# snap-research/MMVID

Hardware: AMD Instinct MI355X
Metric: video-tokens/sec training step, 8-frame 128px text-to-video (higher is better)
Workload: dtype bf16

## Files before the change

mmvid_amd/csrc/attn.hip:

```cpp
#include <type_traits>

#include "../../include/mmvid_hip.h"
#include "gemm_core.h"
#include "prof.h"

namespace {
using mmvid_core::blds16;
using mmvid_core::dma_publish_barrier;
using mmvid_core::make_rsrc;
using mmvid_core::rsrc_t;
using mmvid_core::bf16x4_t;
using mmvid_core::ds_read_tr16;
using mmvid_core::lds_addr;
using mmvid_core::lgkm_wait_tied;
using mmvid_core::xcd_remap;

struct MaskSpec {
    int mode;
    int r0, c0, r1, c1;
};

__device__ __forceinline__ bool is_masked(const MaskSpec& m, int q, int key, int L) {
    const bool pad = key >= L;
    const bool causal = (m.mode == 1) & (key > q);
    const bool rows = (m.mode == 2) & (((q == m.r0) & (key < m.c0)) | ((q == m.r1) & (key < m.c1)));
    return pad | causal | rows;
}

constexpr int TILE = 64 * 128;
constexpr int ROWS_PER_BLOCK = 128;
constexpr float RESCALE_THR = 8.0f;

__device__ __forceinline__ int swz(int row) {
    const int x = (row >> 1) & 7;
    return ((x & 1) << 2) | (x >> 1);
}

struct FastDiv {
    uint32_t d, m;
};
static FastDiv make_fastdiv(int d) {
    FastDiv f;
    f.d = (uint32_t)d, f.m = d > 1 ? (uint32_t)((1ull << 32) / (uint32_t)d) + 1u : 0u;
    return f;
}
__device__ __forceinline__ uint32_t fdiv(uint32_t n, FastDiv f) { return f.d == 1 ? n : __umulhi(n, f.m); }

struct TileStage {
    rsrc_t rsrc;
    uint32_t voff[2], rowbytes;
    __device__ __forceinline__ void init(const bf16_t* slice, long ld, int L, int wave, int lane) {
        rsrc = make_rsrc(slice, (uint32_t)(((long)(L - 1) * ld + 64) * 2));
        rowbytes = (uint32_t)ld * 2u;
#pragma unroll
        for (int jj = 0; jj < 2; ++jj) {
            const int row = (wave * 2 + jj) * 8 + (lane >> 3);
            const int chunk = (lane & 7) ^ swz(row);
            voff[jj] = (uint32_t)row * rowbytes + (uint32_t)chunk * 16u;
        }
    }
    __device__ __forceinline__ void issue(int p0, char* tile, int wave) const {
#pragma unroll
        for (int jj = 0; jj < 2; ++jj) blds16(rsrc, voff[jj], (uint32_t)p0 * rowbytes, tile + (wave * 2 + jj) * 1024);
    }
};

struct RowLane {
    uint32_t o[4];
};
__device__ __forceinline__ RowLane row_lane_offs(int lane) {
    const int l32 = lane & 31, h = lane >> 5;
    RowLane r;
#pragma unroll
    for (int s = 0; s < 4; ++s) r.o[s] = (uint32_t)(l32 * 128 + (((2 * s + h) ^ swz(l32)) << 4));
    return r;
}
template <int SS, int S>
__device__ __forceinline__ bf16x8_t row_frag(const char* tile, const RowLane& rl) {
    return *reinterpret_cast<const bf16x8_t*>(tile + SS * 4096 + rl.o[S]);
}
struct TrLane {
    uint32_t o[2][2];
};
__device__ __forceinline__ TrLane tr_lane_offs(int lane) {
    const int G = lane >> 4, si = lane & 15;
    const int rowl = 4 * (G >> 1) + (si >> 2);
    const int cl = 2 * (G & 1) + ((si & 3) >> 1);
    const int x0 = (rowl >> 1) & 1, x1 = (rowl >> 2) & 1;
    TrLane t;
#pragma unroll
    for (int dt = 0; dt < 2; ++dt)
#pragma unroll
        for (int x2 = 0; x2 < 2; ++x2) t.o[dt][x2] = (uint32_t)(rowl * 128 + ((4 * (dt ^ x0) + (cl ^ x1 ^ (2 * x2))) << 4) + 8 * (si & 1));
    return t;
}
__device__ __forceinline__ TrLane tr_lane_at(const TrLane& t, uint32_t base) {
    TrLane a;
#pragma unroll
    for (int dt = 0; dt < 2; ++dt)
#pragma unroll
        for (int x2 = 0; x2 < 2; ++x2) a.o[dt][x2] = t.o[dt][x2] + base;
    return a;
}
template <int DT, int SS, int M, int OFF>
__device__ __forceinline__ bf16x8_t tr_frag(const TrLane& tl) {
    const bf16x4_t lo = ds_read_tr16<OFF + (32 * SS + 16 * M) * 128>(tl.o[DT][0]);
    const bf16x4_t hi = ds_read_tr16<OFF + (32 * SS + 16 * M + 8) * 128>(tl.o[DT][1]);
    return __builtin_shufflevector(lo, hi, 0, 1, 2, 3, 4, 5, 6, 7);
}
template <int SS, int OFF>
__device__ __forceinline__ void tr_frags4(const TrLane& tl, bf16x8_t (&f)[4]) {
    f[0] = tr_frag<0, SS, 0, OFF>(tl), f[1] = tr_frag<1, SS, 0, OFF>(tl);
    f[2] = tr_frag<0, SS, 1, OFF>(tl), f[3] = tr_frag<1, SS, 1, OFF>(tl);
}
__device__ __forceinline__ bf16x8_t pack_half(const f32x16& a, int m) {
    const int o = 8 * m;
    const uint4 u = make_uint4(pack_bf2(a[o], a[o + 1]), pack_bf2(a[o + 2], a[o + 3]), pack_bf2(a[o + 4], a[o + 5]),
                               pack_bf2(a[o + 6], a[o + 7]));
    return __builtin_bit_cast(bf16x8_t, u);
}
__device__ __forceinline__ f32x16 mfma32(bf16x8_t a, bf16x8_t b, f32x16 c) {
    return __builtin_amdgcn_mfma_f32_32x32x16_bf16(a, b, c, 0, 0, 0);
}
__device__ __forceinline__ f32x16 mfma32z(bf16x8_t a, bf16x8_t b) {
    const f32x16 z = {0.f, 0.f, 0.f, 0.f, 0.f, 0.f, 0.f, 0.f, 0.f, 0.f, 0.f, 0.f, 0.f, 0.f, 0.f, 0.f};
    return __builtin_amdgcn_mfma_f32_32x32x16_bf16(a, b, z, 0, 0, 0);
}
__device__ __forceinline__ f32x16 zero16() {
    f32x16 z;
#pragma unroll
    for (int r = 0; r < 16; ++r) z[r] = 0.f;
    return z;
}
__device__ __forceinline__ constexpr int acc_row(int r, int h) { return (r & 3) + 8 * (r >> 2) + 4 * h; }
__device__ __forceinline__ float fast_exp2(float x) { return __builtin_amdgcn_exp2f(x); }
__device__ __forceinline__ float max16(const f32x16& a) {
    float m0, m1;
    asm("v_max3_f32 %0, %1, %2, %3" : "=v"(m0) : "v"(a[0]), "v"(a[1]), "v"(a[2]));
    asm("v_max3_f32 %0, %1, %2, %3" : "=v"(m1) : "v"(a[3]), "v"(a[4]), "v"(a[5]));
    asm("v_max3_f32 %0, %1, %2, %3" : "=v"(m0) : "v"(m0), "v"(a[6]), "v"(a[7]));
    asm("v_max3_f32 %0, %1, %2, %3" : "=v"(m1) : "v"(m1), "v"(a[8]), "v"(a[9]));
    asm("v_max3_f32 %0, %1, %2, %3" : "=v"(m0) : "v"(m0), "v"(a[10]), "v"(a[11]));
    asm("v_max3_f32 %0, %1, %2, %3" : "=v"(m1) : "v"(m1), "v"(a[12]), "v"(a[13]));
    asm("v_max3_f32 %0, %1, %2, %3" : "=v"(m0) : "v"(m0), "v"(a[14]), "v"(a[15]));
    asm("v_max_f32 %0, %1, %2" : "=v"(m0) : "v"(m0), "v"(m1));
    return m0;
}
__device__ __forceinline__ float half_max(float v) {
    const uint32_t u = __float_as_uint(v);
    const auto r = __builtin_amdgcn_permlane32_swap(u, u, false, false);
    float m;
    asm("v_max_f32 %0, %1, %2" : "=v"(m) : "v"(__uint_as_float(r[0])), "v"(__uint_as_float(r[1])));
    return m;
}
__device__ __forceinline__ float half_sum(float v) {
    const uint32_t u = __float_as_uint(v);
    const auto r = __builtin_amdgcn_permlane32_swap(u, u, false, false);
    return __uint_as_float(r[0]) + __uint_as_float(r[1]);
}
__device__ __forceinline__ float exp2_affine_sum(f32x16& a, float sc, float nb) {
    float s0 = 0.f, s1 = 0.f;
#pragma unroll
    for (int i = 0; i < 8; ++i) {
        float x, y;
        asm("v_fma_f32 %0, %1, %2, %3" : "=v"(x) : "v"(a[2 * i]), "v"(sc), "v"(nb));
        asm("v_fma_f32 %0, %1, %2, %3" : "=v"(y) : "v"(a[2 * i + 1]), "v"(sc), "v"(nb));
        x = fast_exp2(x), y = fast_exp2(y);
        a[2 * i] = x, a[2 * i + 1] = y;
        asm("v_add_f32 %0, %1, %2" : "=v"(s0) : "v"(s0), "v"(x));
        asm("v_add_f32 %0, %1, %2" : "=v"(s1) : "v"(s1), "v"(y));
    }
    return s0 + s1;
}
__device__ __forceinline__ void mask_pad_keys(f32x16& s, int kl) {
#pragma unroll
    for (int r = 0; r < 16; ++r) s[r] = (acc_row(r, 0) >= kl) ? -INFINITY : s[r];
}

__device__ __forceinline__ uint4 widen_pair(uint2 lo, uint2 hi) {
    const auto a = __builtin_amdgcn_permlane32_swap(lo.x, hi.x, false, false);
    const auto b = __builtin_amdgcn_permlane32_swap(lo.y, hi.y, false, false);
    return make_uint4(a[0], b[0], a[1], b[1]);
}
__device__ __forceinline__ void store_row64(bf16_t* row_ptr, const f32x16 (&acc)[2], float scale, int h) {
#pragma unroll
    for (int dt = 0; dt < 2; ++dt)
#pragma unroll
        for (int k = 0; k < 2; ++k) {
            uint2 pc[2];
#pragma unroll
            for (int u = 0; u < 2; ++u) {
                const int g4 = 2 * k + u;
                pc[u] = make_uint2(pack_bf2(acc[dt][4 * g4] * scale, acc[dt][4 * g4 + 1] * scale),
                                   pack_bf2(acc[dt][4 * g4 + 2] * scale, acc[dt][4 * g4 + 3] * scale));
            }
            *reinterpret_cast<uint4*>(row_ptr + 32 * dt + 16 * k + 8 * h) = widen_pair(pc[0], pc[1]);
        }
}

__device__ __forceinline__ void colsum_rows64(const f32x16 (&acc)[2], float scale, bool live, float* dst, int lane) {
    float cs[32];
#pragma unroll
    for (int dt = 0; dt < 2; ++dt)
#pragma unroll
        for (int r = 0; r < 16; ++r) cs[16 * dt + r] = live ? acc[dt][r] * scale : 0.f;
#pragma unroll
    for (int s = 0; s < 5; ++s) {
        const int m = 1 << s;
        const bool up = (lane & m) != 0;
#pragma unroll
        for (int t = 0; t < (16 >> s); ++t) {
            const float keep = up ? cs[2 * t + 1] : cs[2 * t];
            const float send = up ? cs[2 * t] : cs[2 * t + 1];
            cs[t] = keep + __shfl_xor(send, m, 64);
        }
    }
    const int c = lane & 31, h = lane >> 5;
    unsafeAtomicAdd(dst + 32 * (c >> 4) + 8 * ((c >> 2) & 3) + 4 * h + (c & 3), cs[0]);
}

struct BlockCoords {
    int rt, hd, b;
};
__device__ __forceinline__ BlockCoords block_coords(FastDiv nrt, FastDiv H) {
    BlockCoords c;
    const uint32_t id = (uint32_t)xcd_remap(blockIdx.x, gridDim.x);
    const uint32_t bh = fdiv(id, nrt);
    c.rt = (int)(id - bh * nrt.d);
    c.b = (int)fdiv(bh, H);
    c.hd = (int)(bh - (uint32_t)c.b * H.d);
    return c;
}

template <int V>
using ic = std::integral_constant<int, V>;

template <bool KEYLEN>
__global__ __launch_bounds__(256, 3) void attn_fwd_kernel(const bf16_t* __restrict__ qkv, long ld, int L, int H, int E, FastDiv nrt_d,
                                                           FastDiv h_d, float scale_log2, MaskSpec mask, bf16_t* __restrict__ out,
                                                           long ldo, float* __restrict__ lse2, const int32_t* __restrict__ key_len) {
    __shared__ __attribute__((aligned(16))) char smem[2][2 * TILE];
    const int tid = threadIdx.x, lane = tid & 63, wave = __builtin_amdgcn_readfirstlane(tid >> 6), l32 = lane & 31, h = lane >> 5;
    const BlockCoords bc = block_coords(nrt_d, h_d);
    const int qt = bc.rt, hd = bc.hd, b = bc.b;
    const int Lk = KEYLEN ? min(max(key_len[b], 1), L) : L;
    const bf16_t* Kbase = qkv + (long)b * L * ld + E + hd * 64;
    const bf16_t* Vbase = Kbase + E;
    const RowLane rl = row_lane_offs(lane);
    const TrLane trv = tr_lane_at(tr_lane_offs(lane), lds_addr(smem[0] + TILE));
    const int q_wave0 = qt * ROWS_PER_BLOCK + wave * 32;
    const int q = q_wave0 + l32;
    const int qc = q < L ? q : L - 1;
    const bool wave_active = q_wave0 < L;
    bf16x8_t qf[4];
    {
        const bf16_t* Qp = qkv + ((long)b * L + qc) * ld + hd * 64;
#pragma unroll
        for (int s = 0; s < 4; ++s) qf[s] = *reinterpret_cast<const bf16x8_t*>(Qp + 16 * s + 8 * h);
    }
    int kv_end = Lk;
    if (mask.mode == 1) {
        const int blk_end = (qt + 1) * ROWS_PER_BLOCK;
        if (blk_end < L) kv_end = blk_end;
    }
    const int t_begin = 0, t_end = (kv_end + 63) >> 6;

    TileStage stK, stV;
    stK.init(Kbase, ld, Lk, wave, lane), stV.init(Vbase, ld, Lk, wave, lane);
    stK.issue(t_begin * 64, smem[0], wave), stV.issue(t_begin * 64, smem[0] + TILE, wave);

    float m_run = -INFINITY, nref = 0.f, thr_raw = -INFINITY, lsum = 0.f;
    const float inv_scale_log2 = 1.0f / scale_log2;
    f32x16 oacc[2] = {zero16(), zero16()};
    const int row_kmax = mask.mode != 2 ? 0
                                        : max((mask.r0 >= q_wave0 && mask.r0 < q_wave0 + 32) ? mask.c0 : 0,
                                              (mask.r1 >= q_wave0 && mask.r1 < q_wave0 + 32) ? mask.c1 : 0);
    int lo = (row_kmax + 63) >> 6, hi = min(t_end - 1, Lk >> 6);
    if (mask.mode == 1) hi = min(hi, (q_wave0 + 1) >> 6);
    lo = max(lo, t_begin);
    lo += (lo - t_begin) & 1;
    if (lo >= t_end) lo = t_end;
    hi = hi > lo ? lo + ((hi - lo) & ~1) : lo;
    const int kl0 = Lk - 4 * h;

    auto tile = [&](auto st_c, auto plain_c, int t) {
        constexpr int ST = decltype(st_c)::value;
        constexpr bool PLAIN = decltype(plain_c)::value != 0;
        constexpr int VOFF = ST * 2 * TILE;
        const char* Kt = smem[ST];
        char* nxt = smem[ST ^ 1];
        const bool more = PLAIN || t + 1 < t_end;
        const bool two = PLAIN || t * 64 + 32 < Lk;
        f32x16 sv[2];
        auto s_mfmas = [&](auto ss_c) {
            constexpr int SS = decltype(ss_c)::value;
            sv[SS] = mfma32z(row_frag<SS, 0>(Kt, rl), qf[0]);
            sv[SS] = mfma32(row_frag<SS, 1>(Kt, rl), qf[1], sv[SS]);
            sv[SS] = mfma32(row_frag<SS, 2>(Kt, rl), qf[2], sv[SS]);
            sv[SS] = mfma32(row_frag<SS, 3>(Kt, rl), qf[3], sv[SS]);
        };
        s_mfmas(ic<0>{});
        if constexpr (PLAIN) s_mfmas(ic<1>{});
        if (more) {
            __builtin_amdgcn_sched_barrier(0);
            stK.issue((t + 1) * 64, nxt, wave), stV.issue((t + 1) * 64, nxt + TILE, wave);
        }
        auto sub = [&](auto ss_c) {
            constexpr int SS = decltype(ss_c)::value;
            const int key0 = t * 64 + 32 * SS;
            f32x16& s = sv[SS];
            if constexpr (!PLAIN) mfma_settle(s);
            bf16x8_t vt[4];
            tr_frags4<SS, VOFF>(trv, vt);
            if constexpr (!PLAIN) {
                if ((mask.mode == 1 && key0 + 31 > q_wave0) || key0 < row_kmax) {
#pragma unroll
                    for (int r = 0; r < 16; ++r) s[r] = is_masked(mask, q, key0 + acc_row(r, h), Lk) ? -INFINITY : s[r];
                } else if (key0 + 32 > Lk) {
                    mask_pad_keys(s, kl0 - key0);
                }
            }
            const float mx_raw = half_max(max16(s));
            if (__any(mx_raw > thr_raw)) {
                const float m_new = fmaxf(m_run, mx_raw * scale_log2);
                const float m_ref = (m_new == -INFINITY) ? 0.f : m_new;
                const float alpha = fast_exp2(m_run - m_ref);
                lsum *= alpha;
#pragma unroll
                for (int dt = 0; dt < 2; ++dt)
#pragma unroll
                    for (int r = 0; r < 16; ++r) oacc[dt][r] *= alpha;
                m_run = m_new, nref = -m_ref, thr_raw = (m_new + RESCALE_THR) * inv_scale_log2;
            }
            lsum += exp2_affine_sum(s, scale_log2, nref);
            bf16x8_t pf[2] = {pack_half(s, 0), pack_half(s, 1)};
            lgkm_wait_tied<0>(vt[0], vt[1], vt[2], vt[3], pf[0], pf[1]);
            oacc[0] = mfma32(vt[0], pf[0], oacc[0]);
            oacc[1] = mfma32(vt[1], pf[0], oacc[1]);
            oacc[0] = mfma32(vt[2], pf[1], oacc[0]);
            oacc[1] = mfma32(vt[3], pf[1], oacc[1]);
        };
        sub(ic<0>{});
        if (two) {
            if constexpr (!PLAIN) s_mfmas(ic<1>{});
            sub(ic<1>{});
        }
    };
    if (!wave_active) {
        for (int t = t_begin; t < t_end; ++t) {
            dma_publish_barrier();
            char* nxt = smem[(t + 1 - t_begin) & 1];
            if (t + 1 < t_end) stK.issue((t + 1) * 64, nxt, wave), stV.issue((t + 1) * 64, nxt + TILE, wave);
        }
        return;
    }
#pragma unroll 1
    for (int ph = 0; ph < 2; ++ph) {
        const int a = ph == 0 ? t_begin : hi, z = ph == 0 ? lo : t_end;
#pragma unroll 1
        for (int t = a; t < z; ++t) {
            dma_publish_barrier();
            if ((t - t_begin) & 1)
                tile(ic<1>{}, ic<0>{}, t);
            else
                tile(ic<0>{}, ic<0>{}, t);
        }
        if (ph == 0) {
#pragma unroll 1
            for (int t = lo; t < hi; t += 2) {
                dma_publish_barrier();
                tile(ic<0>{}, ic<1>{}, t);
                dma_publish_barrier();
                tile(ic<1>{}, ic<1>{}, t + 1);
            }
        }
    }
    lsum = half_sum(lsum);
    mfma_settle(oacc[0]), mfma_settle(oacc[1]);
    if (q < L) {
        store_row64(out + ((long)b * L + q) * ldo + hd * 64, oacc, 1.0f / lsum, h);
        if (h == 0 && (!KEYLEN || lse2)) lse2[((long)b * H + hd) * L + q] = m_run + log2f(lsum);
    }
}

__global__ __launch_bounds__(256, 3) void attn_bwd_dq_kernel(const bf16_t* __restrict__ qkv, long ld, const bf16_t* __restrict__ O, long ldo,
                                                              const bf16_t* __restrict__ dO, long lddo, const float* __restrict__ lse2,
                                                              float* __restrict__ delta, int L, int H, int E, FastDiv nrt_d, FastDiv h_d,
                                                              float scale, float scale_log2, MaskSpec mask, bf16_t* __restrict__ dqkv,
                                                              long ldg, float* __restrict__ dbias) {
    __shared__ __attribute__((aligned(16))) char smem[2][2 * TILE];
    const int tid = threadIdx.x, lane = tid & 63, wave = __builtin_amdgcn_readfirstlane(tid >> 6), l32 = lane & 31, h = lane >> 5;
    const BlockCoords bc = block_coords(nrt_d, h_d);
    const int qt = bc.rt, hd = bc.hd, b = bc.b;
    const bf16_t* Kbase = qkv + (long)b * L * ld + E + hd * 64;
    const bf16_t* Vbase = Kbase + E;
    const RowLane rl = row_lane_offs(lane);
    const TrLane trk = tr_lane_at(tr_lane_offs(lane), lds_addr(smem[0]));
    const int q_wave0 = qt * ROWS_PER_BLOCK + wave * 32;
    const int q = q_wave0 + l32;
    const int qc = q < L ? q : L - 1;
    const bool wave_active = q_wave0 < L;
    bf16x8_t qf[4], dof[4];
    float neg_lse, my_delta;
    {
        const bf16_t* Qp = qkv + ((long)b * L + qc) * ld + hd * 64;
        const bf16_t* dOp = dO + ((long)b * L + qc) * lddo + hd * 64;
        const bf16_t* Op = O + ((long)b * L + qc) * ldo + hd * 64;
        uint4 o4[4];
#pragma unroll
        for (int s = 0; s < 4; ++s) {
            qf[s] = *reinterpret_cast<const bf16x8_t*>(Qp + 16 * s + 8 * h);
            dof[s] = *reinterpret_cast<const bf16x8_t*>(dOp + 16 * s + 8 * h);
            o4[s] = *reinterpret_cast<const uint4*>(Op + 16 * s + 8 * h);
        }
        neg_lse = -lse2[((long)b * H + hd) * L + qc];
        float d = 0.f;
#pragma unroll
        for (int s = 0; s < 4; ++s) {
            const uint4 d4 = __builtin_bit_cast(uint4, dof[s]);
            d += (bf_lo(o4[s].x) * bf_lo(d4.x) + bf_hi(o4[s].x) * bf_hi(d4.x)) + (bf_lo(o4[s].y) * bf_lo(d4.y) + bf_hi(o4[s].y) * bf_hi(d4.y)) +
                 (bf_lo(o4[s].z) * bf_lo(d4.z) + bf_hi(o4[s].z) * bf_hi(d4.z)) + (bf_lo(o4[s].w) * bf_lo(d4.w) + bf_hi(o4[s].w) * bf_hi(d4.w));
        }
        my_delta = half_sum(d);
        if (h == 0 && q < L) delta[((long)b * H + hd) * L + q] = my_delta;
    }
    int kv_end = L;
    if (mask.mode == 1) {
        const int blk_end = (qt + 1) * ROWS_PER_BLOCK;
        if (blk_end < L) kv_end = blk_end;
    }
    const int t_begin = 0, t_end = (kv_end + 63) >> 6;

    TileStage sk, sv;
    sk.init(Kbase, ld, L, wave, lane), sv.init(Vbase, ld, L, wave, lane);
    sk.issue(t_begin * 64, smem[0], wave), sv.issue(t_begin * 64, smem[0] + TILE, wave);

    f32x16 dq[2] = {zero16(), zero16()};
    const int row_kmax = mask.mode != 2 ? 0
                                        : max((mask.r0 >= q_wave0 && mask.r0 < q_wave0 + 32) ? mask.c0 : 0,
                                              (mask.r1 >= q_wave0 && mask.r1 < q_wave0 + 32) ? mask.c1 : 0);
    int lo = (row_kmax + 63) >> 6, hi = min(t_end - 1, L >> 6);
    if (mask.mode == 1) hi = min(hi, (q_wave0 + 1) >> 6);
    lo = max(lo, t_begin);
    lo += (lo - t_begin) & 1;
    if (lo >= t_end) lo = t_end;
    hi = hi > lo ? lo + ((hi - lo) & ~1) : lo;

    auto tile = [&](auto st_c, auto plain_c, int t) {
        constexpr int ST = decltype(st_c)::value;
        constexpr bool PLAIN = decltype(plain_c)::value != 0;
        constexpr int KOFF = ST * 2 * TILE;
        const char* Kt = smem[ST];
        const char* Vt = Kt + TILE;
        char* nxt = smem[ST ^ 1];
        const bool more = PLAIN || t + 1 < t_end;
        auto sub = [&](auto ss_c) {
            constexpr int SS = decltype(ss_c)::value;
            const int key0 = t * 64 + 32 * SS;
            f32x16 s = mfma32z(row_frag<SS, 0>(Kt, rl), qf[0]);
            f32x16 dp = mfma32z(row_frag<SS, 0>(Vt, rl), dof[0]);
            s = mfma32(row_frag<SS, 1>(Kt, rl), qf[1], s), dp = mfma32(row_frag<SS, 1>(Vt, rl), dof[1], dp);
            s = mfma32(row_frag<SS, 2>(Kt, rl), qf[2], s), dp = mfma32(row_frag<SS, 2>(Vt, rl), dof[2], dp);
            s = mfma32(row_frag<SS, 3>(Kt, rl), qf[3], s), dp = mfma32(row_frag<SS, 3>(Vt, rl), dof[3], dp);
            if (SS == 0 && more) {
                __builtin_amdgcn_sched_barrier(0);
                sk.issue((t + 1) * 64, nxt, wave), sv.issue((t + 1) * 64, nxt + TILE, wave);
            }
            mfma_settle(s), mfma_settle(dp);
            bf16x8_t kt4[4];
            tr_frags4<SS, KOFF>(trk, kt4);
            if constexpr (!PLAIN) {
                if ((mask.mode == 1 && key0 + 31 > q_wave0) || key0 < row_kmax) {
#pragma unroll
                    for (int r = 0; r < 16; ++r) s[r] = is_masked(mask, q, key0 + acc_row(r, h), L) ? -INFINITY : s[r];
                }
                if (key0 + 32 > L) {
#pragma unroll
                    for (int r = 0; r < 16; ++r) s[r] = (key0 + acc_row(r, h) >= L) ? -INFINITY : s[r];
                }
            }
            (void)exp2_affine_sum(s, scale_log2, neg_lse);
#pragma unroll
            for (int r = 0; r < 16; ++r) s[r] *= dp[r] - my_delta;
            bf16x8_t dsf[2] = {pack_half(s, 0), pack_half(s, 1)};
            lgkm_wait_tied<0>(kt4[0], kt4[1], kt4[2], kt4[3], dsf[0], dsf[1]);
            dq[0] = mfma32(kt4[0], dsf[0], dq[0]);
            dq[1] = mfma32(kt4[1], dsf[0], dq[1]);
            dq[0] = mfma32(kt4[2], dsf[1], dq[0]);
            dq[1] = mfma32(kt4[3], dsf[1], dq[1]);
        };
        sub(ic<0>{});
        if (PLAIN || t * 64 + 32 < L) sub(ic<1>{});
    };
    if (!wave_active) {
        for (int t = t_begin; t < t_end; ++t) {
            dma_publish_barrier();
            char* nxt = smem[(t + 1 - t_begin) & 1];
            if (t + 1 < t_end) sk.issue((t + 1) * 64, nxt, wave), sv.issue((t + 1) * 64, nxt + TILE, wave);
        }
        return;
    }
#pragma unroll 1
    for (int ph = 0; ph < 2; ++ph) {
        const int a = ph == 0 ? t_begin : hi, z = ph == 0 ? lo : t_end;
#pragma unroll 1
        for (int t = a; t < z; ++t) {
            dma_publish_barrier();
            if ((t - t_begin) & 1)
                tile(ic<1>{}, ic<0>{}, t);
            else
                tile(ic<0>{}, ic<0>{}, t);
        }
        if (ph == 0) {
#pragma unroll 1
            for (int t = lo; t < hi; t += 2) {
                dma_publish_barrier();
                tile(ic<0>{}, ic<1>{}, t);
                dma_publish_barrier();
                tile(ic<1>{}, ic<1>{}, t + 1);
            }
        }
    }
    mfma_settle(dq[0]), mfma_settle(dq[1]);
    if (q < L) store_row64(dqkv + ((long)b * L + q) * ldg + hd * 64, dq, scale, h);
    if (dbias) colsum_rows64(dq, scale, q < L, dbias + hd * 64, lane);
}

constexpr int DKV_BUF = 2 * TILE + 512;

__global__ __launch_bounds__(256, 2) void attn_bwd_dkv_kernel(const bf16_t* __restrict__ qkv, long ld, const bf16_t* __restrict__ dO, long lddo,
                                                               const float* __restrict__ lse2, const float* __restrict__ delta, int L, int H,
                                                               int E, FastDiv nrt_d, FastDiv h_d, float scale, float scale_log2, MaskSpec mask,
                                                               bf16_t* __restrict__ dqkv, long ldg, float* __restrict__ dbias) {
    __shared__ __attribute__((aligned(16))) char dsm[2][DKV_BUF];
    const int tid = threadIdx.x, lane = tid & 63, wave = __builtin_amdgcn_readfirstlane(tid >> 6), l32 = lane & 31, h = lane >> 5;
    const BlockCoords bc = block_coords(nrt_d, h_d);
    const int kt = bc.rt, hd = bc.hd, b = bc.b;
    const bf16_t* Qbase = qkv + (long)b * L * ld + hd * 64;
    const bf16_t* dObase = dO + (long)b * L * lddo + hd * 64;
    const float* lse_b = lse2 + ((long)b * H + hd) * L;
    const float* del_b = delta + ((long)b * H + hd) * L;
    const int nq_tiles = (L + 63) >> 6;
    const RowLane rl = row_lane_offs(lane);
    const TrLane tr0 = tr_lane_offs(lane);
    const TrLane trq = tr_lane_at(tr0, lds_addr(dsm[0])), trdo = tr_lane_at(tr0, lds_addr(dsm[0] + TILE));
    const int key_wave0 = kt * ROWS_PER_BLOCK + wave * 32;
    const int key = key_wave0 + l32;
    const bool wave_active = key_wave0 < L;
    bf16x8_t kf[4], vf[4];
    {
        const int keyc = key < L ? key : L - 1;
        const bf16_t* Kp = qkv + ((long)b * L + keyc) * ld + E + hd * 64;
        const bf16_t* Vp = Kp + E;
#pragma unroll
        for (int s = 0; s < 4; ++s) {
            kf[s] = *reinterpret_cast<const bf16x8_t*>(Kp + 16 * s + 8 * h);
            vf[s] = *reinterpret_cast<const bf16x8_t*>(Vp + 16 * s + 8 * h);
        }
    }
    auto load_stat = [&](int t) -> float {
        if (tid >= 128) return 0.f;
        const int qq = t * 64 + (tid & 63);
        if (tid < 64) return qq < L ? -lse_b[qq] : -INFINITY;
        return qq < L ? del_b[qq] : 0.f;
    };
    const int t_begin = (mask.mode == 1) ? (kt * ROWS_PER_BLOCK) >> 6 : 0, t_end = nq_tiles;

    TileStage sq, sdo;
    sq.init(Qbase, ld, L, wave, lane), sdo.init(dObase, lddo, L, wave, lane);
    sq.issue(t_begin * 64, dsm[0], wave), sdo.issue(t_begin * 64, dsm[0] + TILE, wave);
    float stat = load_stat(t_begin);
    if (tid < 128) reinterpret_cast<float*>(dsm[0] + 2 * TILE)[tid] = stat;

    f32x16 dk[2] = {zero16(), zero16()}, dv[2] = {zero16(), zero16()};
    const bool rows_hit0 = mask.mode == 2 && key_wave0 < mask.c0, rows_hit1 = mask.mode == 2 && key_wave0 < mask.c1;

    auto tile = [&](auto st_c, int t) {
        constexpr int ST = decltype(st_c)::value;
        constexpr int OFF = ST * DKV_BUF;
        const char* Qt = dsm[ST];
        const char* dOt = Qt + TILE;
        const float* st_nlse = reinterpret_cast<const float*>(Qt + 2 * TILE);
        const float* st_del = st_nlse + 64;
        char* nx = dsm[ST ^ 1];
        const bool more = t + 1 < t_end;
        dma_publish_barrier();
        if (!wave_active) {
            if (more) {
                sq.issue((t + 1) * 64, nx, wave), sdo.issue((t + 1) * 64, nx + TILE, wave);
                stat = load_stat(t + 1);
                if (tid < 128) reinterpret_cast<float*>(nx + 2 * TILE)[tid] = stat;
            }
            return;
        }
        auto sub = [&](auto ss_c) {
            constexpr int SS = decltype(ss_c)::value;
            const int q0 = t * 64 + 32 * SS;
            f32x16 s = mfma32z(row_frag<SS, 0>(Qt, rl), kf[0]);
            f32x16 dp = mfma32z(row_frag<SS, 0>(dOt, rl), vf[0]);
            s = mfma32(row_frag<SS, 1>(Qt, rl), kf[1], s), dp = mfma32(row_frag<SS, 1>(dOt, rl), vf[1], dp);
            s = mfma32(row_frag<SS, 2>(Qt, rl), kf[2], s), dp = mfma32(row_frag<SS, 2>(dOt, rl), vf[2], dp);
            s = mfma32(row_frag<SS, 3>(Qt, rl), kf[3], s), dp = mfma32(row_frag<SS, 3>(dOt, rl), vf[3], dp);
            if (SS == 0 && more) {
                __builtin_amdgcn_sched_barrier(0);
                sq.issue((t + 1) * 64, nx, wave), sdo.issue((t + 1) * 64, nx + TILE, wave);
                stat = load_stat(t + 1);
            }
            mfma_settle(s), mfma_settle(dp);
            bf16x8_t dot4[4], qt4[4];
            tr_frags4<SS, OFF>(trdo, dot4);
            tr_frags4<SS, OFF>(trq, qt4);
            bool nm = mask.mode == 1 && key_wave0 + 31 > q0;
            nm = nm || (rows_hit0 && mask.r0 >= q0 && mask.r0 < q0 + 32) || (rows_hit1 && mask.r1 >= q0 && mask.r1 < q0 + 32);
            if (nm) {
#pragma unroll
                for (int r = 0; r < 16; ++r) s[r] = is_masked(mask, q0 + acc_row(r, h), key, L) ? -INFINITY : s[r];
            }
            const f32x2 sc2 = {scale_log2, scale_log2};
#pragma unroll
            for (int g4 = 0; g4 < 4; ++g4) {
                const int ql = 32 * SS + 8 * g4 + 4 * h;
                const float4 l4 = *reinterpret_cast<const float4*>(st_nlse + ql);
                const float4 d4 = *reinterpret_cast<const float4*>(st_del + ql);
                f32x2 a = {s[4 * g4], s[4 * g4 + 1]}, c = {s[4 * g4 + 2], s[4 * g4 + 3]};
                a = __builtin_elementwise_fma(a, sc2, (f32x2){l4.x, l4.y});
                c = __builtin_elementwise_fma(c, sc2, (f32x2){l4.z, l4.w});
                const float p0 = fast_exp2(a[0]), p1 = fast_exp2(a[1]), p2 = fast_exp2(c[0]), p3 = fast_exp2(c[1]);
                s[4 * g4] = p0, s[4 * g4 + 1] = p1, s[4 * g4 + 2] = p2, s[4 * g4 + 3] = p3;
                dp[4 * g4] = p0 * (dp[4 * g4] - d4.x);
                dp[4 * g4 + 1] = p1 * (dp[4 * g4 + 1] - d4.y);
                dp[4 * g4 + 2] = p2 * (dp[4 * g4 + 2] - d4.z);
                dp[4 * g4 + 3] = p3 * (dp[4 * g4 + 3] - d4.w);
            }
            bf16x8_t pf[2] = {pack_half(s, 0), pack_half(s, 1)};
            bf16x8_t dsf[2] = {pack_half(dp, 0), pack_half(dp, 1)};
            lgkm_wait_tied<8>(dot4[0], dot4[1], dot4[2], dot4[3], pf[0], pf[1]);
            dv[0] = mfma32(dot4[0], pf[0], dv[0]);
            dv[1] = mfma32(dot4[1], pf[0], dv[1]);
            dv[0] = mfma32(dot4[2], pf[1], dv[0]);
            dv[1] = mfma32(dot4[3], pf[1], dv[1]);
            lgkm_wait_tied<0>(qt4[0], qt4[1], qt4[2], qt4[3], dsf[0], dsf[1]);
            dk[0] = mfma32(qt4[0], dsf[0], dk[0]);
            dk[1] = mfma32(qt4[1], dsf[0], dk[1]);
            dk[0] = mfma32(qt4[2], dsf[1], dk[0]);
            dk[1] = mfma32(qt4[3], dsf[1], dk[1]);
        };
        sub(ic<0>{});
        if (t * 64 + 32 < L) sub(ic<1>{});
        if (more && tid < 128) reinterpret_cast<float*>(nx + 2 * TILE)[tid] = stat;
    };
    for (int t = t_begin; t < t_end; t += 2) {
        tile(ic<0>{}, t);
        if (t + 1 >= t_end) break;
        tile(ic<1>{}, t + 1);
    }
    if (!wave_active) return;
    mfma_settle(dk[0]), mfma_settle(dk[1]), mfma_settle(dv[0]), mfma_settle(dv[1]);
    if (key < L) {
        bf16_t* kp = dqkv + ((long)b * L + key) * ldg + E + hd * 64;
        store_row64(kp, dk, scale, h);
        store_row64(kp + E, dv, 1.0f, h);
    }
    if (dbias) {
        colsum_rows64(dk, scale, key < L, dbias + E + hd * 64, lane);
        colsum_rows64(dv, 1.0f, key < L, dbias + 2 * E + hd * 64, lane);
    }
}

static MaskSpec make_mask(int mode, int r0, int c0, int r1, int c1) {
    MaskSpec m;
    m.mode = mode, m.r0 = r0, m.c0 = c0, m.r1 = r1, m.c1 = c1;
    return m;
}

}

#define ATTN_COMMON_CHECKS(name)                                                                            \
    MMVID_REQUIRE(B > 0 && L > 0 && H > 0 && E == H * 64, name ": need E == H*64 (head_dim 64), got E=%d H=%d", E, H); \
    MMVID_REQUIRE(mask_mode >= 0 && mask_mode <= 2, name ": mask_mode %d", mask_mode);                             \
    MMVID_REQUIRE((int64_t)cdiv(L, ROWS_PER_BLOCK) * H * B * (H > 64 ? H : 64) < (1ll << 31), name ": too many (batch, head, row block) units")

extern "C" int mmvid_attention_fwd(const void* qkv, int64_t ld, int B, int L, int H, int E, float scale, int mask_mode,
                                   int r0, int c0, int r1, int c1, void* out, int64_t ldo, float* lse2, void* stream) {
    MMVID_REQUIRE(qkv && out && lse2, "attention_fwd: null pointer");
    ATTN_COMMON_CHECKS("attention_fwd");
    MMVID_REQUIRE(ld % 8 == 0 && ldo % 8 == 0 && ((uintptr_t)out & 15) == 0, "attention_fwd: leading dims must be multiples of 8, out 16-byte aligned");
    MMVID_REQUIRE((int64_t)L * ld * 2 < (1ll << 31), "attention_fwd: one batch entry of qkv must be smaller than 2 GiB");
    hipStream_t s = (hipStream_t)stream;
    MmvidProfScope prof(PROF_ATTN_FWD, 4.0 * B * H * (double)L * L * 64, s);
    const int nrt = cdiv(L, ROWS_PER_BLOCK), nblocks = nrt * H * B;
    const FastDiv nrt_d = make_fastdiv(nrt), h_d = make_fastdiv(H);
    const MaskSpec m = make_mask(mask_mode, r0, c0, r1, c1);
    hipLaunchKernelGGL(attn_fwd_kernel<false>, dim3(nblocks), dim3(256), 0, s, (const bf16_t*)qkv, (long)ld, L, H, E, nrt_d, h_d,
                       scale * 1.4426950408889634f, m, (bf16_t*)out, (long)ldo, lse2, (const int32_t*)nullptr);
    MMVID_LAUNCH_CHECK("attention_fwd");
    return MMVID_OK;
}

extern "C" int mmvid_attention_fwd_keylen(const void* qkv, int64_t ld, int B, int L, int H, int E, float scale, const int32_t* key_len,
                                          void* out, int64_t ldo, float* lse2, void* stream) {
    MMVID_REQUIRE(qkv && out && key_len, "attention_fwd_keylen: null pointer");
    const int mask_mode = 0;
    ATTN_COMMON_CHECKS("attention_fwd_keylen");
    MMVID_REQUIRE(ld % 8 == 0 && ldo % 8 == 0 && ((uintptr_t)out & 15) == 0,
                  "attention_fwd_keylen: leading dims must be multiples of 8, out 16-byte aligned");
    MMVID_REQUIRE((int64_t)L * ld * 2 < (1ll << 31), "attention_fwd_keylen: one batch entry of qkv must be smaller than 2 GiB");
    hipStream_t s = (hipStream_t)stream;
    MmvidProfScope prof(PROF_ATTN_FWD, 4.0 * B * H * (double)L * L * 64, s);
    const int nrt = cdiv(L, ROWS_PER_BLOCK), nblocks = nrt * H * B;
    const FastDiv nrt_d = make_fastdiv(nrt), h_d = make_fastdiv(H);
    hipLaunchKernelGGL(attn_fwd_kernel<true>, dim3(nblocks), dim3(256), 0, s, (const bf16_t*)qkv, (long)ld, L, H, E, nrt_d, h_d,
                       scale * 1.4426950408889634f, make_mask(0, -1, 0, -1, 0), (bf16_t*)out, (long)ldo, lse2, key_len);
    MMVID_LAUNCH_CHECK("attention_fwd_keylen");
    return MMVID_OK;
}

extern "C" int mmvid_attention_bwd(const void* qkv, int64_t ld, const void* O, int64_t ldo, const void* dO, int64_t lddo,
                                   const float* lse2, float* delta, int B, int L, int H, int E, float scale,
                                   int mask_mode, int r0, int c0, int r1, int c1, void* dqkv, int64_t ldg,
                                   void* stream) {
    return mmvid_attention_bwd_bias(qkv, ld, O, ldo, dO, lddo, lse2, delta, B, L, H, E, scale, mask_mode, r0, c0, r1, c1, dqkv, ldg,
                                    nullptr, stream);
}

extern "C" int mmvid_attention_bwd_bias(const void* qkv, int64_t ld, const void* O, int64_t ldo, const void* dO, int64_t lddo,
                                        const float* lse2, float* delta, int B, int L, int H, int E, float scale,
                                        int mask_mode, int r0, int c0, int r1, int c1, void* dqkv, int64_t ldg,
                                        float* dbias, void* stream) {
    MMVID_REQUIRE(qkv && O && dO && lse2 && delta && dqkv, "attention_bwd: null pointer");
    ATTN_COMMON_CHECKS("attention_bwd");
    MMVID_REQUIRE(ld % 8 == 0 && ldo % 8 == 0 && lddo % 8 == 0 && ldg % 8 == 0 && ((uintptr_t)dqkv & 15) == 0,
                  "attention_bwd: leading dims must be multiples of 8, dqkv 16-byte aligned");
    MMVID_REQUIRE((int64_t)L * ld * 2 < (1ll << 31) && (int64_t)L * lddo * 2 < (1ll << 31),
                  "attention_bwd: one batch entry of qkv / dO must be smaller than 2 GiB");
    hipStream_t s = (hipStream_t)stream;
    const MaskSpec m = make_mask(mask_mode, r0, c0, r1, c1);
    const float sl2 = scale * 1.4426950408889634f;
    MmvidProfScope prof(PROF_ATTN_BWD, 10.0 * B * H * (double)L * L * 64, s);
    const int nrt = cdiv(L, ROWS_PER_BLOCK), nblocks = nrt * H * B;
    const FastDiv nrt_d = make_fastdiv(nrt), h_d = make_fastdiv(H);
    hipLaunchKernelGGL(attn_bwd_dq_kernel, dim3(nblocks), dim3(256), 0, s, (const bf16_t*)qkv, (long)ld, (const bf16_t*)O, (long)ldo,
                       (const bf16_t*)dO, (long)lddo, lse2, delta, L, H, E, nrt_d, h_d, scale, sl2, m, (bf16_t*)dqkv, (long)ldg, dbias);
    hipLaunchKernelGGL(attn_bwd_dkv_kernel, dim3(nblocks), dim3(256), 0, s, (const bf16_t*)qkv, (long)ld, (const bf16_t*)dO, (long)lddo, lse2,
                       delta, L, H, E, nrt_d, h_d, scale, sl2, m, (bf16_t*)dqkv, (long)ldg, dbias);
    MMVID_LAUNCH_CHECK("attention_bwd");
    return MMVID_OK;
}
```

Baseline: 215,900.

## Fold softmax stats into MFMA accumulator init and raise dkv occupancy

The dK/dV backward kernel now seeds the S and dP MFMA accumulators with the per-row -lse/scale and -delta values. The exponent then becomes a single multiply and exp, and dS becomes a single multiply, which removes the per-element FMA/subtract work and the separate stat loads in the inner loop. Launch bounds go from 2 to 3 blocks per SIMD, the Q-transpose read is deferred to cut register pressure, and the tile-stage DMA uses one offset register for two 32-row halves. The risks are inline asm scheduling (s_nop hazard handling), register spills at the higher occupancy target, and a small precision change from dividing lse by scale.

```diff
diff --git a/mmvid_amd/csrc/attn.hip b/mmvid_amd/csrc/attn.hip
--- a/mmvid_amd/csrc/attn.hip
+++ b/mmvid_amd/csrc/attn.hip
@@ -48,20 +48,17 @@
 
 struct TileStage {
     rsrc_t rsrc;
-    uint32_t voff[2], rowbytes;
+    uint32_t voff, rowbytes;
     __device__ __forceinline__ void init(const bf16_t* slice, long ld, int L, int wave, int lane) {
         rsrc = make_rsrc(slice, (uint32_t)(((long)(L - 1) * ld + 64) * 2));
         rowbytes = (uint32_t)ld * 2u;
-#pragma unroll
-        for (int jj = 0; jj < 2; ++jj) {
-            const int row = (wave * 2 + jj) * 8 + (lane >> 3);
-            const int chunk = (lane & 7) ^ swz(row);
-            voff[jj] = (uint32_t)row * rowbytes + (uint32_t)chunk * 16u;
-        }
+        const int row = wave * 8 + (lane >> 3);
+        const int chunk = (lane & 7) ^ swz(row);
+        voff = (uint32_t)row * rowbytes + (uint32_t)chunk * 16u;
     }
     __device__ __forceinline__ void issue(int p0, char* tile, int wave) const {
-#pragma unroll
-        for (int jj = 0; jj < 2; ++jj) blds16(rsrc, voff[jj], (uint32_t)p0 * rowbytes, tile + (wave * 2 + jj) * 1024);
+        blds16(rsrc, voff, (uint32_t)p0 * rowbytes, tile + wave * 1024);
+        blds16(rsrc, voff, (uint32_t)(p0 + 32) * rowbytes, tile + (wave + 4) * 1024);
     }
 };
 
@@ -528,10 +525,22 @@
 
 constexpr int DKV_BUF = 2 * TILE + 512;
 
-__global__ __launch_bounds__(256, 2) void attn_bwd_dkv_kernel(const bf16_t* __restrict__ qkv, long ld, const bf16_t* __restrict__ dO, long lddo,
+template <int SS>
+__device__ __forceinline__ f32x16 row_consts(const float* st, int h) {
+    f32x16 a;
+#pragma unroll
+    for (int g4 = 0; g4 < 4; ++g4) {
+        const float4 v = *reinterpret_cast<const float4*>(st + 32 * SS + 8 * g4 + 4 * h);
+        a[4 * g4] = v.x, a[4 * g4 + 1] = v.y, a[4 * g4 + 2] = v.z, a[4 * g4 + 3] = v.w;
+    }
+    return a;
+}
+
+__global__ __launch_bounds__(256, 3) void attn_bwd_dkv_kernel(const bf16_t* __restrict__ qkv, long ld, const bf16_t* __restrict__ dO, long lddo,
                                                                const float* __restrict__ lse2, const float* __restrict__ delta, int L, int H,
-                                                               int E, FastDiv nrt_d, FastDiv h_d, float scale, float scale_log2, MaskSpec mask,
-                                                               bf16_t* __restrict__ dqkv, long ldg, float* __restrict__ dbias) {
+                                                               int E, FastDiv nrt_d, FastDiv h_d, float scale, float scale_log2,
+                                                               float inv_scale_log2, MaskSpec mask, bf16_t* __restrict__ dqkv, long ldg,
+                                                               float* __restrict__ dbias) {
     __shared__ __attribute__((aligned(16))) char dsm[2][DKV_BUF];
     const int tid = threadIdx.x, lane = tid & 63, wave = __builtin_amdgcn_readfirstlane(tid >> 6), l32 = lane & 31, h = lane >> 5;
     const BlockCoords bc = block_coords(nrt_d, h_d);
@@ -542,8 +551,7 @@
     const float* del_b = delta + ((long)b * H + hd) * L;
     const int nq_tiles = (L + 63) >> 6;
     const RowLane rl = row_lane_offs(lane);
-    const TrLane tr0 = tr_lane_offs(lane);
-    const TrLane trq = tr_lane_at(tr0, lds_addr(dsm[0])), trdo = tr_lane_at(tr0, lds_addr(dsm[0] + TILE));
+    const TrLane trq = tr_lane_at(tr_lane_offs(lane), lds_addr(dsm[0]));
     const int key_wave0 = kt * ROWS_PER_BLOCK + wave * 32;
     const int key = key_wave0 + l32;
     const bool wave_active = key_wave0 < L;
@@ -561,8 +569,8 @@
     auto load_stat = [&](int t) -> float {
         if (tid >= 128) return 0.f;
         const int qq = t * 64 + (tid & 63);
-        if (tid < 64) return qq < L ? -lse_b[qq] : -INFINITY;
-        return qq < L ? del_b[qq] : 0.f;
+        if (tid < 64) return qq < L ? -lse_b[qq] * inv_scale_log2 : -INFINITY;
+        return qq < L ? -del_b[qq] : 0.f;
     };
     const int t_begin = (mask.mode == 1) ? (kt * ROWS_PER_BLOCK) >> 6 : 0, t_end = nq_tiles;
 
@@ -581,7 +589,7 @@
         const char* Qt = dsm[ST];
         const char* dOt = Qt + TILE;
         const float* st_nlse = reinterpret_cast<const float*>(Qt + 2 * TILE);
-        const float* st_del = st_nlse + 64;
+        const float* st_ndel = st_nlse + 64;
         char* nx = dsm[ST ^ 1];
         const bool more = t + 1 < t_end;
         dma_publish_barrier();
@@ -596,8 +604,8 @@
         auto sub = [&](auto ss_c) {
             constexpr int SS = decltype(ss_c)::value;
             const int q0 = t * 64 + 32 * SS;
-            f32x16 s = mfma32z(row_frag<SS, 0>(Qt, rl), kf[0]);
-            f32x16 dp = mfma32z(row_frag<SS, 0>(dOt, rl), vf[0]);
+            f32x16 s = row_consts<SS>(st_nlse, h), dp = row_consts<SS>(st_ndel, h);
+            s = mfma32(row_frag<SS, 0>(Qt, rl), kf[0], s), dp = mfma32(row_frag<SS, 0>(dOt, rl), vf[0], dp);
             s = mfma32(row_frag<SS, 1>(Qt, rl), kf[1], s), dp = mfma32(row_frag<SS, 1>(dOt, rl), vf[1], dp);
             s = mfma32(row_frag<SS, 2>(Qt, rl), kf[2], s), dp = mfma32(row_frag<SS, 2>(dOt, rl), vf[2], dp);
             s = mfma32(row_frag<SS, 3>(Qt, rl), kf[3], s), dp = mfma32(row_frag<SS, 3>(dOt, rl), vf[3], dp);
@@ -607,33 +615,26 @@
                 stat = load_stat(t + 1);
             }
             mfma_settle(s), mfma_settle(dp);
-            bf16x8_t dot4[4], qt4[4];
-            tr_frags4<SS, OFF>(trdo, dot4);
-            tr_frags4<SS, OFF>(trq, qt4);
+            bf16x8_t dot4[4];
+            tr_frags4<SS, OFF + TILE>(trq, dot4);
             bool nm = mask.mode == 1 && key_wave0 + 31 > q0;
             nm = nm || (rows_hit0 && mask.r0 >= q0 && mask.r0 < q0 + 32) || (rows_hit1 && mask.r1 >= q0 && mask.r1 < q0 + 32);
             if (nm) {
 #pragma unroll
                 for (int r = 0; r < 16; ++r) s[r] = is_masked(mask, q0 + acc_row(r, h), key, L) ? -INFINITY : s[r];
             }
-            const f32x2 sc2 = {scale_log2, scale_log2};
-#pragma unroll
-            for (int g4 = 0; g4 < 4; ++g4) {
-                const int ql = 32 * SS + 8 * g4 + 4 * h;
-                const float4 l4 = *reinterpret_cast<const float4*>(st_nlse + ql);
-                const float4 d4 = *reinterpret_cast<const float4*>(st_del + ql);
-                f32x2 a = {s[4 * g4], s[4 * g4 + 1]}, c = {s[4 * g4 + 2], s[4 * g4 + 3]};
-                a = __builtin_elementwise_fma(a, sc2, (f32x2){l4.x, l4.y});
-                c = __builtin_elementwise_fma(c, sc2, (f32x2){l4.z, l4.w});
-                const float p0 = fast_exp2(a[0]), p1 = fast_exp2(a[1]), p2 = fast_exp2(c[0]), p3 = fast_exp2(c[1]);
-                s[4 * g4] = p0, s[4 * g4 + 1] = p1, s[4 * g4 + 2] = p2, s[4 * g4 + 3] = p3;
-                dp[4 * g4] = p0 * (dp[4 * g4] - d4.x);
-                dp[4 * g4 + 1] = p1 * (dp[4 * g4 + 1] - d4.y);
-                dp[4 * g4 + 2] = p2 * (dp[4 * g4 + 2] - d4.z);
-                dp[4 * g4 + 3] = p3 * (dp[4 * g4 + 3] - d4.w);
+#pragma unroll
+            for (int r = 0; r < 16; ++r) {
+                float p, ds;
+                asm("v_mul_f32 %0, %2, %3\n\tv_exp_f32 %0, %0\n\ts_nop 0\n\tv_mul_f32 %1, %0, %4"
+                    : "=&v"(p), "=&v"(ds)
+                    : "v"(s[r]), "v"(scale_log2), "v"(dp[r]));
+                s[r] = p, dp[r] = ds;
             }
             bf16x8_t pf[2] = {pack_half(s, 0), pack_half(s, 1)};
             bf16x8_t dsf[2] = {pack_half(dp, 0), pack_half(dp, 1)};
+            bf16x8_t qt4[4];
+            tr_frags4<SS, OFF>(trq, qt4);
             lgkm_wait_tied<8>(dot4[0], dot4[1], dot4[2], dot4[3], pf[0], pf[1]);
             dv[0] = mfma32(dot4[0], pf[0], dv[0]);
             dv[1] = mfma32(dot4[1], pf[0], dv[1]);
@@ -656,14 +657,15 @@
     }
     if (!wave_active) return;
     mfma_settle(dk[0]), mfma_settle(dk[1]), mfma_settle(dv[0]), mfma_settle(dv[1]);
-    if (key < L) {
-        bf16_t* kp = dqkv + ((long)b * L + key) * ldg + E + hd * 64;
-        store_row64(kp, dk, scale, h);
-        store_row64(kp + E, dv, 1.0f, h);
+    const int lane_e = (int)__lane_id(), key_e = key_wave0 + (lane_e & 31), h_e = lane_e >> 5;
+    if (key_e < L) {
+        bf16_t* kp = dqkv + ((long)b * L + key_e) * ldg + E + hd * 64;
+        store_row64(kp, dk, scale, h_e);
+        store_row64(kp + E, dv, 1.0f, h_e);
     }
     if (dbias) {
-        colsum_rows64(dk, scale, key < L, dbias + E + hd * 64, lane);
-        colsum_rows64(dv, 1.0f, key < L, dbias + 2 * E + hd * 64, lane);
+        colsum_rows64(dk, scale, key_e < L, dbias + E + hd * 64, lane_e);
+        colsum_rows64(dv, 1.0f, key_e < L, dbias + 2 * E + hd * 64, lane_e);
     }
 }
 
@@ -742,7 +744,7 @@
     hipLaunchKernelGGL(attn_bwd_dq_kernel, dim3(nblocks), dim3(256), 0, s, (const bf16_t*)qkv, (long)ld, (const bf16_t*)O, (long)ldo,
                        (const bf16_t*)dO, (long)lddo, lse2, delta, L, H, E, nrt_d, h_d, scale, sl2, m, (bf16_t*)dqkv, (long)ldg, dbias);
     hipLaunchKernelGGL(attn_bwd_dkv_kernel, dim3(nblocks), dim3(256), 0, s, (const bf16_t*)qkv, (long)ld, (const bf16_t*)dO, (long)lddo, lse2,
-                       delta, L, H, E, nrt_d, h_d, scale, sl2, m, (bf16_t*)dqkv, (long)ldg, dbias);
+                       delta, L, H, E, nrt_d, h_d, scale, sl2, 1.0f / sl2, m, (bf16_t*)dqkv, (long)ldg, dbias);
     MMVID_LAUNCH_CHECK("attention_bwd");
     return MMVID_OK;
 }
```

Result: faster. 219,300, median of 6 (+1.5%).
